# PKU-Alignment/Safe-Policy-Optimization

Hardware: NVIDIA H100
Metric: env-steps/sec PPO-Lag SafetyPointGoal1 @1024 envs/GPU (higher is better)
Workload: dtype f32

## Files before the change

### safe-policy-optimization_b200/csrc/spo_update_kernel.cuh

```cuda
#pragma once
#include <cooperative_groups.h>
#include <stdlib.h>
#include "spo_common.cuh"
#include "spo_mma.cuh"

namespace cg = cooperative_groups;

int spo_update_tile_pool(cudaMemPool_t* pool);

#ifdef SPO_PHASE_TIMERS
__device__ unsigned long long g_phase_cycles[16][24];
#define PHASE_MARK(idx)                                                   \
  do {                                                                    \
    if (tid == 0) {                                                       \
      const long long now__ = clock64();                                  \
      sm_phase__[idx] += static_cast<unsigned long long>(now__ - phase_t__); \
      phase_t__ = now__;                                                  \
    }                                                                     \
  } while (0)
#else
#define PHASE_MARK(idx) do { } while (0)
#endif

namespace {

constexpr int UT = 256;
constexpr int NQ = 4;
constexpr int SL = SPO_HID / NQ;
constexpr int NCTA = 3 * NQ;
constexpr int LDA = 72;
constexpr int LDS = 40;
constexpr float kLogSqrt2Pi = 0.91893853320467274178f;

template <int AC>
struct UpdShape {
  static_assert(AC == 8 || AC == 16, "action capacity 8 or 16");
  static constexpr int AUXW = 3 * AC + 4;
  static constexpr int AUX_LOGP = AC, AUX_ADV = AC + 1, AUX_TGT = AC + 2, AUX_OMEAN = AC + 4, AUX_OSTD = 2 * AC + 4;
  static constexpr int SP_B1 = 0, SP_B2 = SL, SP_W3 = 2 * SL, SP_B3 = 2 * SL + AC * SL, SP_LS = SP_B3 + AC;
  static constexpr int SPN = SP_LS + AC;
  static constexpr int SPT = (SPN + UT - 1) / UT;
  static constexpr int YQ = SPO_ROWS * AC;
  static constexpr int DH = AC / 4;
};
static_assert(UpdShape<8>::SPN == 176 && UpdShape<8>::SPT == 1 && UpdShape<16>::SPN == 320 && UpdShape<16>::SPT == 2, "layout");

__host__ __device__ constexpr int upd_ldx(int nt1) { return 64 * nt1 + 8; }
template <int NT1, int AC>
__host__ __device__ constexpr int upd_tile_floats() { return SPO_ROWS * (upd_ldx(NT1) + UpdShape<AC>::AUXW); }
static_assert(upd_tile_floats<1, 8>() * 4 == 25600 && upd_tile_floats<2, 8>() * 4 == 41984 && upd_tile_floats<2, 16>() * 4 % 16 == 0,
              "bulk copies move multiples of 16 bytes");
__host__ __device__ constexpr int dp_slot_words(int nt1) { return UT * 4 * (1 + nt1) + UT; }

template <int N> struct IC { static constexpr int value = N; };

struct UpdArgs {
  float *params, *adam_m, *adam_v;
  int* adam_t;
  float* tiles;
  spo_batch data;
  const int64_t* perm;
  int64_t perm_len;
  int batch, kind, D, A;
  int actor_only;
  spo_hparams hp;
  spo_update_ctrl* ctrl;
  spo_comm comm;
};

__device__ __forceinline__ uint32_t smem_u32(const void* p) { return static_cast<uint32_t>(__cvta_generic_to_shared(p)); }
__device__ __forceinline__ uint32_t mapa(uint32_t addr, uint32_t rank) {
  uint32_t r;
  asm volatile("mapa.shared::cluster.u32 %0, %1, %2;" : "=r"(r) : "r"(addr), "r"(rank));
  return r;
}
__device__ __forceinline__ void mbar_init(uint64_t* bar, uint32_t count) {
  asm volatile("mbarrier.init.shared::cta.b64 [%0], %1;" ::"r"(smem_u32(bar)), "r"(count) : "memory");
}
__device__ __forceinline__ void mbar_expect_tx(uint64_t* bar, uint32_t bytes) {
  asm volatile("mbarrier.arrive.expect_tx.shared::cta.b64 _, [%0], %1;" ::"r"(smem_u32(bar)), "r"(bytes) : "memory");
}
__device__ __forceinline__ void mbar_wait(uint64_t* bar, uint32_t parity) {
  const uint32_t a = smem_u32(bar);
  uint32_t ok = 0;
  while (!ok) {
    asm volatile("{ .reg .pred p; mbarrier.try_wait.parity.shared::cta.b64 p, [%1], %2; selp.u32 %0, 1, 0, p; }"
                 : "=r"(ok) : "r"(a), "r"(parity) : "memory");
  }
}
__device__ __forceinline__ void mbar_wait_cluster(uint64_t* bar, uint32_t parity) {
  const uint32_t a = smem_u32(bar);
  uint32_t ok = 0;
  while (!ok) {
    asm volatile("{ .reg .pred p; mbarrier.try_wait.parity.acquire.cluster.shared::cta.b64 p, [%1], %2; selp.u32 %0, 1, 0, p; }"
                 : "=r"(ok) : "r"(a), "r"(parity) : "memory");
  }
}
__device__ __forceinline__ void st_async16(uint32_t remote_dst, float4 v, uint32_t remote_bar) {
  asm volatile("st.async.shared::cluster.mbarrier::complete_tx::bytes.v4.b32 [%0], {%1, %2, %3, %4}, [%5];"
               ::"r"(remote_dst), "r"(__float_as_uint(v.x)), "r"(__float_as_uint(v.y)), "r"(__float_as_uint(v.z)),
               "r"(__float_as_uint(v.w)), "r"(remote_bar) : "memory");
}
__device__ __forceinline__ void bulk_push(uint32_t remote_dst, const void* local_src, uint32_t bytes, uint32_t remote_bar) {
  asm volatile("cp.async.bulk.shared::cluster.shared::cta.mbarrier::complete_tx::bytes [%0], [%1], %2, [%3];"
               ::"r"(remote_dst), "r"(smem_u32(local_src)), "r"(bytes), "r"(remote_bar) : "memory");
}
__device__ __forceinline__ void fence_proxy_async() { asm volatile("fence.proxy.async.shared::cta;" ::: "memory"); }
__device__ __forceinline__ void bulk_load(void* smem_dst, const void* gmem_src, uint32_t bytes, uint64_t* bar) {
  asm volatile("cp.async.bulk.shared::cluster.global.mbarrier::complete_tx::bytes [%0], [%1], %2, [%3];"
               ::"r"(smem_u32(smem_dst)), "l"(gmem_src), "r"(bytes), "r"(smem_u32(bar)) : "memory");
}
__device__ __forceinline__ void bulk_prefetch_l2(const void* gmem_src, uint32_t bytes) {
  asm volatile("cp.async.bulk.prefetch.L2.global [%0], %1;" ::"l"(gmem_src), "r"(bytes) : "memory");
}
__device__ __forceinline__ void st_ll(float2* p, float v, unsigned seq) {
  asm volatile("st.relaxed.sys.global.v2.b32 [%0], {%1, %2};" ::"l"(p), "r"(__float_as_uint(v)), "r"(seq) : "memory");
}

struct AdamK {
  float w1, b2, w2, ibc2s, eps, ss;
};
__device__ __forceinline__ float sqrt_approx(float x) {
  float r;
  asm("sqrt.approx.f32 %0, %1;" : "=f"(r) : "f"(x));
  return r;
}
__device__ __forceinline__ float adam_update(float p, float g, float& m, float& v, const AdamK& k) {
  m = fmaf(k.w1, __fsub_rn(g, m), m);
  v = __fadd_rn(__fmul_rn(v, k.b2), __fmul_rn(__fmul_rn(k.w2, g), g));
  const float denom = fmaf(sqrt_approx(v), k.ibc2s, k.eps);
  return __fadd_rn(p, __fdividef(__fmul_rn(k.ss, m), denom));
}

template <int NTL, int KSTEPS, bool ACCUM>
__device__ __forceinline__ void warp_gemm(float (&acc)[NTL][4], const float* __restrict__ A, int a_sm, int a_sk,
                                          const float* __restrict__ B, int b_sk, int b_sn, int m0, int n0) {
  const int lane = threadIdx.x & 31, g = lane >> 2, t = lane & 3;
  const float* a_ptr = A + (m0 + g) * a_sm + t * a_sk;
  const float* b_ptr = B + t * b_sk + (n0 + g) * b_sn;
  float c_lh[NTL][4], c_hl[NTL][4], c_hh[NTL][4];
#pragma unroll
  for (int nt = 0; nt < NTL; ++nt)
#pragma unroll
    for (int e = 0; e < 4; ++e) { c_lh[nt][e] = 0.f; c_hl[nt][e] = 0.f; c_hh[nt][e] = 0.f; }
  constexpr int CH = KSTEPS < 8 ? KSTEPS : 8;
#pragma unroll
  for (int kc = 0; kc < KSTEPS; kc += CH) {
    float af[CH][4], bf[CH][NTL][2];
#pragma unroll
    for (int ks = 0; ks < CH; ++ks) {
      const float* p = a_ptr + (kc + ks) * 8 * a_sk;
      af[ks][0] = p[0]; af[ks][1] = p[8 * a_sm]; af[ks][2] = p[4 * a_sk]; af[ks][3] = p[8 * a_sm + 4 * a_sk];
#pragma unroll
      for (int nt = 0; nt < NTL; ++nt) {
        const float* pb = b_ptr + nt * 8 * b_sn + (kc + ks) * 8 * b_sk;
        bf[ks][nt][0] = pb[0]; bf[ks][nt][1] = pb[4 * b_sk];
      }
    }
#pragma unroll
    for (int ks = 0; ks < CH; ++ks) {
      uint32_t ah[4], al[4];
#pragma unroll
      for (int i = 0; i < 4; ++i) spo_split_tf32(af[ks][i], ah[i], al[i]);
#pragma unroll
      for (int nt = 0; nt < NTL; ++nt) {
        uint32_t bh[2], bl[2];
        spo_split_tf32(bf[ks][nt][0], bh[0], bl[0]);
        spo_split_tf32(bf[ks][nt][1], bh[1], bl[1]);
        spo_mma_tf32(c_lh[nt], al, bh);
        spo_mma_tf32(c_hl[nt], ah, bl);
        spo_mma_tf32(c_hh[nt], ah, bh);
      }
    }
  }
#pragma unroll
  for (int nt = 0; nt < NTL; ++nt)
#pragma unroll
    for (int e = 0; e < 4; ++e) {
      const float s = (c_lh[nt][e] + c_hl[nt][e]) + c_hh[nt][e];
      acc[nt][e] = ACCUM ? acc[nt][e] + s : s;
    }
}

template <int KSTEPS>
__device__ __forceinline__ void warp_gemm_kk(float (&acc)[1][4], const float* __restrict__ A, int lda,
                                             const float* __restrict__ B, int ldb, int m0, int n0) {
  const int lane = threadIdx.x & 31, g = lane >> 2, t = lane & 3;
  const float* a_ptr = A + (m0 + g) * lda + 2 * t;
  const float* b_ptr = B + (n0 + g) * ldb + 2 * t;
  float c_lh[4] = {0.f, 0.f, 0.f, 0.f}, c_hl[4] = {0.f, 0.f, 0.f, 0.f}, c_hh[4] = {0.f, 0.f, 0.f, 0.f};
  constexpr int CH = KSTEPS < 8 ? KSTEPS : 8;
#pragma unroll
  for (int kc = 0; kc < KSTEPS; kc += CH) {
    float2 a0[CH], a1[CH], bb[CH];
#pragma unroll
    for (int ks = 0; ks < CH; ++ks) {
      a0[ks] = *reinterpret_cast<const float2*>(a_ptr + (kc + ks) * 8);
      a1[ks] = *reinterpret_cast<const float2*>(a_ptr + 8 * lda + (kc + ks) * 8);
      bb[ks] = *reinterpret_cast<const float2*>(b_ptr + (kc + ks) * 8);
    }
#pragma unroll
    for (int ks = 0; ks < CH; ++ks) {
      uint32_t ah[4], al[4], bh[2], bl[2];
      spo_split_tf32(a0[ks].x, ah[0], al[0]);
      spo_split_tf32(a1[ks].x, ah[1], al[1]);
      spo_split_tf32(a0[ks].y, ah[2], al[2]);
      spo_split_tf32(a1[ks].y, ah[3], al[3]);
      spo_split_tf32(bb[ks].x, bh[0], bl[0]);
      spo_split_tf32(bb[ks].y, bh[1], bl[1]);
      spo_mma_tf32(c_lh, al, bh);
      spo_mma_tf32(c_hl, ah, bl);
      spo_mma_tf32(c_hh, ah, bh);
    }
  }
#pragma unroll
  for (int e = 0; e < 4; ++e) acc[0][e] = (c_lh[e] + c_hl[e]) + c_hh[e];
}

constexpr int H1Q = SPO_ROWS * SL;

__device__ __forceinline__ void warp_gemm_l2(float (&acc)[1][4], const float* __restrict__ h1, const float* __restrict__ B, int ldb, int m0, int n0) {
  const int lane = threadIdx.x & 31, g = lane >> 2, t = lane & 3;
  const int r0 = m0 + g, sw = ((r0 >> 1) & 1) << 3;
  const float* b_ptr = B + (n0 + g) * ldb + 2 * t;
  float c_lh[4] = {0.f, 0.f, 0.f, 0.f}, c_hl[4] = {0.f, 0.f, 0.f, 0.f}, c_hh[4] = {0.f, 0.f, 0.f, 0.f};
  float2 a0[8], a1[8], bb[8];
#pragma unroll
  for (int ks = 0; ks < 8; ++ks) {
    const float* blk = h1 + (ks >> 1) * H1Q + ((((ks & 1) << 3) + 2 * t) ^ sw);
    a0[ks] = *reinterpret_cast<const float2*>(blk + r0 * SL);
    a1[ks] = *reinterpret_cast<const float2*>(blk + (r0 + 8) * SL);
    bb[ks] = *reinterpret_cast<const float2*>(b_ptr + ks * 8);
  }
#pragma unroll
  for (int ks = 0; ks < 8; ++ks) {
    uint32_t ah[4], al[4], bh[2], bl[2];
    spo_split_tf32(a0[ks].x, ah[0], al[0]);
    spo_split_tf32(a1[ks].x, ah[1], al[1]);
    spo_split_tf32(a0[ks].y, ah[2], al[2]);
    spo_split_tf32(a1[ks].y, ah[3], al[3]);
    spo_split_tf32(bb[ks].x, bh[0], bl[0]);
    spo_split_tf32(bb[ks].y, bh[1], bl[1]);
    spo_mma_tf32(c_lh, al, bh);
    spo_mma_tf32(c_hl, ah, bl);
    spo_mma_tf32(c_hh, ah, bh);
  }
#pragma unroll
  for (int e = 0; e < 4; ++e) acc[0][e] = (c_lh[e] + c_hl[e]) + c_hh[e];
}

__device__ __forceinline__ void warp_gemm_dw2(float (&acc)[1][4], const float* __restrict__ dz, int ldz, const float* __restrict__ h1, int n0) {
  const int lane = threadIdx.x & 31, g = lane >> 2, t = lane & 3;
  const float* a_ptr = dz + t * ldz + g;
  const int n = n0 + g, sw = ((t >> 1) & 1) << 3;
  const float* b_ptr = h1 + (n >> 4) * H1Q + t * SL + ((n & 15) ^ sw);
  float c_lh[4] = {0.f, 0.f, 0.f, 0.f}, c_hl[4] = {0.f, 0.f, 0.f, 0.f}, c_hh[4] = {0.f, 0.f, 0.f, 0.f};
  float af[8][4], bf[8][2];
#pragma unroll
  for (int ks = 0; ks < 8; ++ks) {
    const float* p = a_ptr + ks * 8 * ldz;
    af[ks][0] = p[0]; af[ks][1] = p[8]; af[ks][2] = p[4 * ldz]; af[ks][3] = p[4 * ldz + 8];
    const float* pb = b_ptr + ks * 8 * SL;
    bf[ks][0] = pb[0]; bf[ks][1] = pb[4 * SL];
  }
#pragma unroll
  for (int ks = 0; ks < 8; ++ks) {
    uint32_t ah[4], al[4], bh[2], bl[2];
#pragma unroll
    for (int i = 0; i < 4; ++i) spo_split_tf32(af[ks][i], ah[i], al[i]);
    spo_split_tf32(bf[ks][0], bh[0], bl[0]);
    spo_split_tf32(bf[ks][1], bh[1], bl[1]);
    spo_mma_tf32(c_lh, al, bh);
    spo_mma_tf32(c_hl, ah, bl);
    spo_mma_tf32(c_hh, ah, bh);
  }
#pragma unroll
  for (int e = 0; e < 4; ++e) acc[0][e] += (c_lh[e] + c_hl[e]) + c_hh[e];
}

template <int NT1, int AC>
__host__ __device__ constexpr size_t update_fixed_smem_bytes() {
  using S = UpdShape<AC>;
  return sizeof(float) * (4 * AC + 16 + SL * upd_ldx(NT1) + SL * LDA + 2 * S::SPN + NQ * SPO_ROWS * SL + 3 * SPO_ROWS * LDS +
                          (3 + NQ) * SPO_ROWS * AC + 2 * NQ * SPO_ROWS * SL + 64 + 128 + 3 * (4 * NT1 + 1) * UT);
}
template <int NT1, int AC>
__host__ __device__ constexpr int update_nslot() {
  return update_fixed_smem_bytes<NT1, AC>() + 2 * sizeof(float) * upd_tile_floats<NT1, AC>() <= 227 * 1024 ? 2 : 1;
}
template <int NT1, int AC>
__host__ __device__ constexpr size_t update_smem_bytes() {
  return update_fixed_smem_bytes<NT1, AC>() + update_nslot<NT1, AC>() * sizeof(float) * upd_tile_floats<NT1, AC>();
}
static_assert(update_smem_bytes<1, 8>() == 172352 && update_smem_bytes<2, 8>() == 221504 && update_smem_bytes<1, 16>() == 200256 &&
              update_smem_bytes<2, 16>() == 201280, "shared-memory figures in the comment above");

template <int NT1, int AC>
__global__ void __launch_bounds__(256) spo_pack_tiles(const UpdArgs a, int64_t n_tiles) {
  using S = UpdShape<AC>;
  if (*reinterpret_cast<volatile int*>(&a.ctrl->stop)) return;
  constexpr int ldx = upd_ldx(NT1), AUXW = S::AUXW, TILEF = upd_tile_floats<NT1, AC>();
  const int D = a.D, A = a.A, lane = threadIdx.x & 31;
  const int tps = (a.batch + SPO_ROWS - 1) / SPO_ROWS;
  const bool actor = a.kind != SPO_LOSS_CRITIC_ONLY, focops = a.kind == SPO_LOSS_FOCOPS;
  const int64_t n_rows = n_tiles * SPO_ROWS, wstride = (static_cast<int64_t>(gridDim.x) * blockDim.x) >> 5;
  for (int64_t w = (static_cast<int64_t>(blockIdx.x) * blockDim.x + threadIdx.x) >> 5; w < n_rows; w += wstride) {
    const int64_t t = w / SPO_ROWS, step = t / tps;
    const int r = static_cast<int>(w - t * SPO_ROWS), row = static_cast<int>(t - step * tps) * SPO_ROWS + r;
    int64_t rows_step = a.perm_len - step * a.batch;
    if (rows_step > a.batch) rows_step = a.batch;
    const bool valid = row < rows_step;
    const int64_t g = valid ? a.perm[step * a.batch + row] : 0;
    float* xo = a.tiles + t * TILEF + r * ldx;
    float* ao = a.tiles + t * TILEF + SPO_ROWS * ldx + r * AUXW;
    const float* xs = a.data.obs + g * D;
    for (int c = lane; c < ldx; c += 32) xo[c] = (valid && c < D) ? xs[c] : 0.f;
    for (int c = lane; c < AUXW; c += 32) {
      const float* src = nullptr;
      int64_t i = g;
      if (c < A) { if (actor) { src = a.data.act; i = g * A + c; } }
      else if (c == S::AUX_LOGP) { if (actor) src = a.data.logp; }
      else if (c == S::AUX_ADV) { if (actor) src = a.data.adv; }
      else if (c == S::AUX_TGT) src = a.data.target_r;
      else if (c == S::AUX_TGT + 1) src = a.data.target_c;
      else if (c >= S::AUX_OMEAN && c < S::AUX_OMEAN + A) { if (focops) { src = a.data.old_mean; i = g * A + c - S::AUX_OMEAN; } }
      else if (c >= S::AUX_OSTD && c < S::AUX_OSTD + A) { if (focops) { src = a.data.old_std; i = g * A + c - S::AUX_OSTD; } }
      ao[c] = (valid && src) ? src[i] : 0.f;
    }
  }
}

template <int NT1, int AC, bool DP>
__global__ void __launch_bounds__(UT, 1) spo_update_kernel(const UpdArgs a) {
  static_assert(!(DP && AC != 8), "the cross-GPU gradient slots hold one small parameter per thread");
  using S = UpdShape<AC>;
  constexpr int AUXW = S::AUXW, AUX_LOGP = S::AUX_LOGP, AUX_ADV = S::AUX_ADV, AUX_TGT = S::AUX_TGT, AUX_OMEAN = S::AUX_OMEAN,
                AUX_OSTD = S::AUX_OSTD;
  constexpr int SP_B1 = S::SP_B1, SP_B2 = S::SP_B2, SP_W3 = S::SP_W3, SP_B3 = S::SP_B3, SP_LS = S::SP_LS, SPN = S::SPN;
  constexpr int SPT = S::SPT, YQ = S::YQ, DH = S::DH;
  constexpr int NSLOT = update_nslot<NT1, AC>(), TILEF = upd_tile_floats<NT1, AC>();
  constexpr uint32_t TILEB = TILEF * sizeof(float);
  extern __shared__ __align__(16) float smem[];
  __shared__ __align__(8) uint64_t bar_h1, bar_dh, bar_y, bar_ss[2];
  __shared__ __align__(8) uint64_t bar_tile[NSLOT];
  __shared__ int comm_dead;
  cg::cluster_group cluster = cg::this_cluster();
  const unsigned rank = cluster.block_rank();
  const int tid = threadIdx.x, lane = tid & 31, wid = tid >> 5;
  spo_update_ctrl* ctrl = a.ctrl;
  if (*reinterpret_cast<volatile int*>(&ctrl->stop)) return;

  const int D = a.D, A = a.A;
  constexpr int ldx = upd_ldx(NT1);
  const bool idle = rank >= NCTA;
  const int net = idle ? 2 : static_cast<int>(rank) / NQ;
  const int q = static_cast<int>(rank) % NQ;
  const unsigned grp0 = static_cast<unsigned>(net * NQ);
  const bool is_actor = (net == 0);
  const bool active = !idle && !(is_actor && a.kind == SPO_LOSS_CRITIC_ONLY) && !(!is_actor && a.actor_only);
  const SpoNetOff off = spo_net_off(D, A, net);
  const int O = off.out;
  const int g8 = lane >> 2, t4 = lane & 3;

  float* p = smem;
  float* lsc = p; p += 4 * AC;
  float* adk = p; p += 16;
  float* w1s = p; p += SL * ldx;
  float* w2s = p; p += SL * LDA;
  float* sp = p;  p += SPN;
  float* gsmall = p; p += SPN;
  float* slots = p; p += NSLOT * TILEF;
  float* x = slots;
  float* aux = x + SPO_ROWS * ldx;
  float* h1 = p;  p += NQ * H1Q;
  float* h2s = p; p += SPO_ROWS * LDS;
  float* dz2s = p; p += SPO_ROWS * LDS;
  float* dz1s = p; p += SPO_ROWS * LDS;
  float* yblk = p; p += NQ * YQ;
  float* y = p;   p += SPO_ROWS * AC;
  float* dy = p;  p += SPO_ROWS * AC;
  float* dls = p; p += SPO_ROWS * AC;
  float* dh1b = p; p += NQ * H1Q;
  float* dh1in = p; p += NQ * H1Q;
  float* red = p; p += 64;
  float* bk = p;  p += 3 * (4 * NT1 + 1) * UT;
  float* xin = p; p += 2 * 16 * 4;
  float* b1s = sp + SP_B1; float* b2s = sp + SP_B2; float* w3s = sp + SP_W3; float* b3 = sp + SP_B3; float* log_std = sp + SP_LS;

  const int tps = (a.batch + SPO_ROWS - 1) / SPO_ROWS;
  const int64_t n_steps = (a.perm_len + a.batch - 1) / a.batch;
  const int64_t n_tiles = n_steps * tps;
  auto issue_tile = [&](int64_t t) {
    if (t >= n_tiles) return;
    const int s = static_cast<int>(t % NSLOT);
    mbar_expect_tx(&bar_tile[s], TILEB);
    bulk_load(slots + s * TILEF, a.tiles + t * TILEF, TILEB, &bar_tile[s]);
    if (NSLOT == 1 && t + 1 < n_tiles) bulk_prefetch_l2(a.tiles + (t + 1) * TILEF, TILEB);
  };

  if (tid == 0) {
    comm_dead = 0;
    mbar_init(&bar_h1, 1);
    mbar_init(&bar_dh, 1);
    mbar_init(&bar_y, 1);
    mbar_init(&bar_ss[0], 1);
    mbar_init(&bar_ss[1], 1);
#pragma unroll
    for (int s = 0; s < NSLOT; ++s) mbar_init(&bar_tile[s], 1);
    asm volatile("fence.mbarrier_init.release.cluster;" ::: "memory");
    if (!idle) { mbar_expect_tx(&bar_ss[0], (NCTA - 1) * 16); mbar_expect_tx(&bar_ss[1], (NCTA - 1) * 16); }
    for (int b = 0; b < 2; ++b) {
      adk[8 * b + 0] = static_cast<float>(1.0 - static_cast<double>(a.hp.beta1));
      adk[8 * b + 1] = a.hp.beta2;
      adk[8 * b + 2] = static_cast<float>(1.0 - static_cast<double>(a.hp.beta2));
      adk[8 * b + 4] = a.hp.adam_eps;
    }
    if (active) {
      mbar_expect_tx(&bar_h1, (NQ - 1) * H1Q * 4);
      mbar_expect_tx(&bar_dh, (NQ - 1) * H1Q * 4);
      mbar_expect_tx(&bar_y, (NQ - 1) * YQ * 4);
#pragma unroll
      for (int t = 0; t < NSLOT; ++t) issue_tile(t);
    }
  }

  bool sp_valid = false, sp_counted = false;
  int sp_goff = 0;
  if (tid < SPN && !idle) {
    const int i = tid;
    sp_counted = true;
    if (i < SP_B2) { sp_valid = true; sp_goff = off.b1 + SL * q + i; }
    else if (i < SP_W3) { sp_valid = true; sp_goff = off.b2 + SL * q + (i - SP_B2); }
    else if (i < SP_B3) { const int o = (i - SP_W3) / SL, kk = (i - SP_W3) % SL; sp_valid = o < O; sp_goff = off.w3 + o * SPO_HID + SL * q + kk; }
    else if (i < SP_LS) { const int o = i - SP_B3; sp_valid = o < O; sp_goff = off.b3 + o; sp_counted = (q == 0); }
    else { const int j = i - SP_LS; sp_valid = is_actor && j < A; sp_goff = off.log_std + j; sp_counted = (q == 0); }
  }
  float sp_m = 0.f, sp_v = 0.f;
  bool sp_valid1 = false, sp_counted1 = false;
  int sp_goff1 = 0;
  float sp_m1 = 0.f, sp_v1 = 0.f;
  if constexpr (SPT > 1) {
    static_assert(UT > SP_W3, "entry 1 lies past b1 / b2");
    const int i = tid + UT;
    if (i < SPN && !idle) {
      sp_counted1 = true;
      if (i < SP_B3) { const int o = (i - SP_W3) / SL, kk = (i - SP_W3) % SL; sp_valid1 = o < O; sp_goff1 = off.w3 + o * SPO_HID + SL * q + kk; }
      else if (i < SP_LS) { const int o = i - SP_B3; sp_valid1 = o < O; sp_goff1 = off.b3 + o; sp_counted1 = (q == 0); }
      else { const int j = i - SP_LS; sp_valid1 = is_actor && j < A; sp_goff1 = off.log_std + j; sp_counted1 = (q == 0); }
    }
  }

  if (!idle) {
    for (int i = tid; i < SL * ldx; i += UT) {
      const int j = i / ldx, k = i - j * ldx;
      w1s[i] = (k < D) ? __ldg(a.params + off.w1 + (SL * q + j) * D + k) : 0.f;
    }
    for (int i = tid; i < SL * LDA; i += UT) {
      const int j = i / LDA, k = i - j * LDA;
      w2s[i] = (k < SPO_HID) ? __ldg(a.params + off.w2 + (SL * q + j) * SPO_HID + k) : 0.f;
    }
    if (tid < SPN) {
      sp[tid] = sp_valid ? a.params[sp_goff] : 0.f;
      gsmall[tid] = 0.f;
      if (sp_valid) { sp_m = a.adam_m[sp_goff]; sp_v = a.adam_v[sp_goff]; }
    }
    if constexpr (SPT > 1) {
      if (tid + UT < SPN) {
        sp[tid + UT] = sp_valid1 ? a.params[sp_goff1] : 0.f;
        gsmall[tid + UT] = 0.f;
        if (sp_valid1) { sp_m1 = a.adam_m[sp_goff1]; sp_v1 = a.adam_v[sp_goff1]; }
      }
    }
  }
  float mW2[4], vW2[4], mW1[NT1][4], vW1[NT1][4];
  auto frag_jk = [&](int e, int ntile, int& j, int& k) { j = g8 + ((e >> 1) << 3); k = 8 * ntile + 2 * t4 + (e & 1); };
#pragma unroll
  for (int e = 0; e < 4; ++e) {
    int j, k;
    frag_jk(e, wid, j, k);
    mW2[e] = active ? a.adam_m[off.w2 + (SL * q + j) * SPO_HID + k] : 0.f;
    vW2[e] = active ? a.adam_v[off.w2 + (SL * q + j) * SPO_HID + k] : 0.f;
#pragma unroll
    for (int i = 0; i < NT1; ++i) {
      frag_jk(e, wid + 8 * i, j, k);
// ... 177 lines not shown
        vW1[i][e] = bk[(2 * NWB + 4 * i + e) * UT + tid];
      }
    }
    if (tid < SP_B2) {
      sp[tid] = bk[(0 * NWB + NWB - 1) * UT + tid];
      sp_m = bk[(1 * NWB + NWB - 1) * UT + tid];
      sp_v = bk[(2 * NWB + NWB - 1) * UT + tid];
    }
  };
  auto clear_l1_grads = [&]() {
#pragma unroll
    for (int e = 0; e < 4; ++e)
#pragma unroll
      for (int i = 0; i < NT1; ++i) gW1[i][e] = 0.f;
    if (tid < SP_B2) gsmall[tid] = 0.f;
  };
  auto set_lsc = [&](int j, float ls) {
    const float sd = expf(ls);
    lsc[4 * j + 0] = sd;
    lsc[4 * j + 1] = __fdiv_rn(1.f, __fmul_rn(sd, sd));
    lsc[4 * j + 2] = logf(sd);
  };
  auto adam_rest = [&](float clip, const AdamK& k) {
    float2 w2v[2];
    float spv = 0.f, spg = 0.f, spv1 = 0.f, spg1 = 0.f;
    const bool own0 = tid >= SP_B2 && tid < SPN;
#pragma unroll
    for (int e = 0; e < 4; e += 2) {
      int j, kc;
      frag_jk(e, wid, j, kc);
      w2v[e >> 1] = *reinterpret_cast<const float2*>(w2s + j * LDA + kc);
    }
    if (own0) { spv = sp[tid]; spg = gsmall[tid]; }
    if constexpr (SPT > 1) {
      if (tid + UT < SPN) { spv1 = sp[tid + UT]; spg1 = gsmall[tid + UT]; }
    }
#pragma unroll
    for (int e = 0; e < 4; e += 2) {
      w2v[e >> 1].x = adam_update(w2v[e >> 1].x, __fmul_rn(gW2[0][e], clip), mW2[e], vW2[e], k);
      w2v[e >> 1].y = adam_update(w2v[e >> 1].y, __fmul_rn(gW2[0][e + 1], clip), mW2[e + 1], vW2[e + 1], k);
    }
    if (own0 && sp_valid) {
      spv = adam_update(spv, __fmul_rn(spg, clip), sp_m, sp_v, k);
      if (tid >= SP_LS) set_lsc(tid - SP_LS, spv);
    }
    if constexpr (SPT > 1) {
      if (tid + UT < SPN && sp_valid1) {
        spv1 = adam_update(spv1, __fmul_rn(spg1, clip), sp_m1, sp_v1, k);
        if (tid + UT >= SP_LS) set_lsc(tid + UT - SP_LS, spv1);
      }
    }
#pragma unroll
    for (int e = 0; e < 4; e += 2) {
      int j, kc;
      frag_jk(e, wid, j, kc);
      *reinterpret_cast<float2*>(w2s + j * LDA + kc) = w2v[e >> 1];
    }
    if (own0) { sp[tid] = spv; gsmall[tid] = 0.f; }
    if constexpr (SPT > 1) {
      if (tid + UT < SPN) { sp[tid + UT] = spv1; gsmall[tid + UT] = 0.f; }
    }
#pragma unroll
    for (int e = 0; e < 4; ++e) gW2[0][e] = 0.f;
  };

  int64_t step = 0;
  int sub = 0;
  auto next_tile = [&]() { if (++sub == tps) { sub = 0; ++step; } };
  for (int64_t qt = 0; qt < n_tiles; ++qt, next_tile()) {
    x = slots + (qt % NSLOT) * TILEF;
    aux = x + SPO_ROWS * ldx;
    int64_t rs64 = a.perm_len - step * a.batch;
    if (rs64 > a.batch) rs64 = a.batch;
    const int rows_step = static_cast<int>(rs64);
    int rows = rows_step - sub * SPO_ROWS;
    rows = rows < 0 ? 0 : (rows > SPO_ROWS ? SPO_ROWS : rows);
    const bool last_tile = (sub == tps - 1);
    const float inv_b = __fdiv_rn(1.f, static_cast<float>(rows_step));
    const unsigned seq = static_cast<unsigned>(a.comm.seq_base + static_cast<unsigned long long>(step_idx) + 1ull);
    const int par = static_cast<int>(step_idx & 1);
    auto dp_push = [&](const float* vals, auto n_c, int w0) {
      constexpr int n = decltype(n_c)::value;
      const size_t base = ((static_cast<size_t>(seq & 1u) * world + me) * NCTA + rank) * DPW;
      for (int r = 0; r < world; ++r) {
        if (r == me) continue;
        float2* dst = reinterpret_cast<float2*>(a.comm.grad_bufs[r]) + base;
#pragma unroll
        for (int i = 0; i < n; ++i) st_ll(dst + (w0 + i) * UT + tid, vals[i], seq);
      }
    };
    auto dp_sum_wide = [&](float (&g2)[4], float (&g1)[NT1][4], float& gs) {
      constexpr int NW = 4 * (1 + NT1) + 1, G = 3;
      const unsigned limit = a.comm.spin_limit ? a.comm.spin_limit : 400000000u;
      const float inv_w = __fdiv_rn(1.f, static_cast<float>(world));
      float val[NW];
#pragma unroll
      for (int e = 0; e < 4; ++e) {
        val[e] = g2[e];
#pragma unroll
        for (int i = 0; i < NT1; ++i) val[4 * (1 + i) + e] = g1[i][e];
      }
      val[NW - 1] = gs;
      const float2* slot0 = reinterpret_cast<const float2*>(a.comm.grad_bufs[me]) + (static_cast<size_t>(seq & 1u) * world * NCTA + rank) * DPW + tid;
      const size_t rstride = static_cast<size_t>(NCTA) * DPW;
#pragma unroll
      for (int i0 = 0; i0 < NW; i0 += G) {
        unsigned need = 0;
#pragma unroll
        for (int j = 0; j < G; ++j)
          if (i0 + j < NW && ((i0 + j < NW - 1) || tid < SPN))
#pragma unroll
            for (int r = 0; r < 8; ++r)
              if (r < world && r != me) need |= 1u << (r * G + j);
        unsigned got = 0, polls = 0;
        float v[8][G];
        while (got != need) {
          unsigned wa[8][G], wb[8][G];
#pragma unroll
          for (int r = 0; r < 8; ++r)
#pragma unroll
            for (int j = 0; j < G; ++j)
              if (((need & ~got) >> (r * G + j)) & 1u)
                asm volatile("ld.relaxed.sys.global.v2.b32 {%0, %1}, [%2];" : "=r"(wa[r][j]), "=r"(wb[r][j]) : "l"(slot0 + r * rstride + (i0 + j) * UT) : "memory");
#pragma unroll
          for (int r = 0; r < 8; ++r)
#pragma unroll
            for (int j = 0; j < G; ++j)
              if ((((need & ~got) >> (r * G + j)) & 1u) && wb[r][j] == seq) { v[r][j] = __uint_as_float(wa[r][j]); got |= 1u << (r * G + j); }
          if (got != need) {
            if (*reinterpret_cast<volatile int*>(&comm_dead)) break;
            if (++polls > limit) { comm_dead = 1; atomicExch(&ctrl->stop, 2); break; }
          }
        }
#pragma unroll
        for (int j = 0; j < G; ++j)
          if (i0 + j < NW) {
            float acc = 0.f;
#pragma unroll
            for (int r = 0; r < 8; ++r)
              if (r < world) acc += (r == me) ? val[i0 + j] : (((got >> (r * G + j)) & 1u) ? v[r][j] : 0.f);
            val[i0 + j] = __fmul_rn(acc, inv_w);
          }
      }
#pragma unroll
      for (int e = 0; e < 4; ++e) {
        g2[e] = val[e];
#pragma unroll
        for (int i = 0; i < NT1; ++i) g1[i][e] = val[4 * (1 + i) + e];
      }
      gs = val[NW - 1];
    };
    auto dp_sum_all = [&](float (&g2)[4], float (&g1)[NT1][4], float& gs) {
      constexpr int NW = 4 * (1 + NT1) + 1;
      const unsigned limit = a.comm.spin_limit ? a.comm.spin_limit : 400000000u;
      const unsigned need = (tid < SPN) ? ((1u << NW) - 1u) : ((1u << (NW - 1)) - 1u);
      float acc[NW];
#pragma unroll
      for (int i = 0; i < NW; ++i) acc[i] = 0.f;
      for (int r = 0; r < world; ++r) {
        if (r == me) {
#pragma unroll
          for (int e = 0; e < 4; ++e) {
            acc[e] += g2[e];
#pragma unroll
            for (int i = 0; i < NT1; ++i) acc[4 * (1 + i) + e] += g1[i][e];
          }
          acc[NW - 1] += gs;
          continue;
        }
        const float2* src = reinterpret_cast<const float2*>(a.comm.grad_bufs[me]) + ((static_cast<size_t>(seq & 1u) * world + r) * NCTA + rank) * DPW + tid;
        unsigned got = 0, polls = 0;
        float v[NW];
#pragma unroll
        for (int i = 0; i < NW; ++i) v[i] = 0.f;
        while (got != need) {
          unsigned wa[NW], wb[NW];
#pragma unroll
          for (int i = 0; i < NW; ++i)
            if (!((got >> i) & 1u) && ((need >> i) & 1u))
              asm volatile("ld.relaxed.sys.global.v2.b32 {%0, %1}, [%2];" : "=r"(wa[i]), "=r"(wb[i]) : "l"(src + i * UT) : "memory");
#pragma unroll
          for (int i = 0; i < NW; ++i)
            if (!((got >> i) & 1u) && ((need >> i) & 1u) && wb[i] == seq) { v[i] = __uint_as_float(wa[i]); got |= 1u << i; }
          if (got != need) {
            if (*reinterpret_cast<volatile int*>(&comm_dead)) break;
            if (++polls > limit) { comm_dead = 1; atomicExch(&ctrl->stop, 2); break; }
          }
        }
#pragma unroll
        for (int i = 0; i < NW; ++i) acc[i] += v[i];
      }
      const float inv_w = __fdiv_rn(1.f, static_cast<float>(world));
#pragma unroll
      for (int e = 0; e < 4; ++e) {
        g2[e] = __fmul_rn(acc[e], inv_w);
#pragma unroll
        for (int i = 0; i < NT1; ++i) g1[i][e] = __fmul_rn(acc[4 * (1 + i) + e], inv_w);
      }
      gs = __fmul_rn(acc[NW - 1], inv_w);
    };

    if (active) mbar_wait(&bar_tile[qt % NSLOT], static_cast<uint32_t>(qt / NSLOT) & 1u);
    __syncthreads();
    PHASE_MARK(0);

    if (active) layer1();
    PHASE_MARK(2);
    const bool defer = pending;
    float clip = 1.f;
    if (pending) {
      pending = false;
      step_barrier_wait();
      PHASE_MARK(9);
      clip = resolve_clip(pend_par);
      if (active) {
        if (clip < 1.f) {
          __syncthreads();
          adam_l1_restore();
          adam_l1(clip, false, adam_k(pend_par));
          __syncthreads();
          layer1();
        }
        clear_l1_grads();
      }
    }
    PHASE_MARK(1);
    float yv[AC];
    if (active) {
      __syncthreads();
      if (lane == 0 && wid < NQ && wid != q)
        bulk_push(mapa(smem_u32(h1 + q * H1Q), grp0 + wid), h1 + q * H1Q, H1Q * 4, mapa(smem_u32(&bar_h1), grp0 + wid));
      if (defer) {
        adam_rest(clip, adam_k(pend_par));
        __syncthreads();
      } else if (qt == 0 && is_actor && tid >= UT - 32 && tid - (UT - 32) < A) {
        set_lsc(tid - (UT - 32), log_std[tid - (UT - 32)]);
      }
      PHASE_MARK(19);
      mbar_wait(&bar_h1, ph_x);
      if (tid == 0) mbar_expect_tx(&bar_h1, (NQ - 1) * H1Q * 4);
      PHASE_MARK(3);
      {
        float acc[1][4];
        warp_gemm_l2(acc, h1, w2s, LDA, mt * 16, ntl * 8);
        const float2 bb = *reinterpret_cast<const float2*>(b2s + cA);
        *reinterpret_cast<float2*>(h2s + rA * LDS + cA) = make_float2(spo_tanh_fast(acc[0][0] + bb.x), spo_tanh_fast(acc[0][1] + bb.y));
        *reinterpret_cast<float2*>(h2s + (rA + 8) * LDS + cA) = make_float2(spo_tanh_fast(acc[0][2] + bb.x), spo_tanh_fast(acc[0][3] + bb.y));
      }
      __syncthreads();
      {
        const float4 hv = *reinterpret_cast<const float4*>(h2s + r4 * LDS + 4 * k4);
        for (int o = 0; o < O; o += 2) {
          const float4 wa = *reinterpret_cast<const float4*>(w3s + o * SL + 4 * k4);
          const float4 wb = *reinterpret_cast<const float4*>(w3s + (o + 1) * SL + 4 * k4);
          float sa = fmaf(hv.x, wa.x, hv.y * wa.y) + fmaf(hv.z, wa.z, hv.w * wa.w);
          float sb = fmaf(hv.x, wb.x, hv.y * wb.y) + fmaf(hv.z, wb.z, hv.w * wb.w);
          sa += __shfl_xor_sync(0xffffffffu, sa, 1);
          sb += __shfl_xor_sync(0xffffffffu, sb, 1);
          sa += __shfl_xor_sync(0xffffffffu, sa, 2);
          sb += __shfl_xor_sync(0xffffffffu, sb, 2);
          if (k4 == (o & 3)) yblk[q * YQ + r4 * AC + o] = sa;
          if (k4 == ((o + 1) & 3) && o + 1 < O) yblk[q * YQ + r4 * AC + o + 1] = sb;
        }
        fence_proxy_async();
      }
      __syncthreads();
      if (lane == 0 && wid < NQ && wid != q)
        bulk_push(mapa(smem_u32(yblk + q * YQ), grp0 + wid), yblk + q * YQ, YQ * 4, mapa(smem_u32(&bar_y), grp0 + wid));
      PHASE_MARK(4);
      float pa[DH], psd[DH], piv[DH], pls[DH], plogp = 0.f, padv = 0.f, ptgt = 0.f;
#pragma unroll
      for (int h = 0; h < DH; ++h) pa[h] = 0.f;
#pragma unroll
      for (int h = 0; h < DH; ++h) psd[h] = 1.f;
#pragma unroll
      for (int h = 0; h < DH; ++h) piv[h] = 1.f;
#pragma unroll
      for (int h = 0; h < DH; ++h) pls[h] = 0.f;
      {
        const float* axp = aux + r4 * AUXW;
        if (is_actor) {
#pragma unroll
          for (int h = 0; h < DH; ++h) {
            const int j = k4 + 4 * h;
            if (j < A) { pa[h] = axp[j]; psd[h] = lsc[4 * j]; piv[h] = lsc[4 * j + 1]; pls[h] = lsc[4 * j + 2]; }
          }
          plogp = axp[AUX_LOGP];
          padv = axp[AUX_ADV];
        } else if (k4 == 0) {
          ptgt = axp[AUX_TGT + (net == 2 ? 1 : 0)];
        }
      }
      if (defer) log_loss(pend_par, pend_inv_b);
      if (last_tile) {
        float* kp = adk + 8 * par;
        if (tid == UT - 32) {
          b1pow *= static_cast<double>(a.hp.beta1);
          kp[5] = -__fdiv_rn(lr, static_cast<float>(1.0 - b1pow));
        } else if (tid == UT - 64) {
          b2pow *= static_cast<double>(a.hp.beta2);
          kp[3] = __fdiv_rn(1.f, sqrtf(static_cast<float>(1.0 - b2pow)));
        }
      }
      mbar_wait(&bar_y, ph_x);
      if (tid == 0) mbar_expect_tx(&bar_y, (NQ - 1) * YQ * 4);
      PHASE_MARK(5);
      {
        const float4* yp = reinterpret_cast<const float4*>(yblk + k4 * YQ + r4 * AC);
#pragma unroll
        for (int c = 0; c < AC / 4; ++c) {
          float4 v = make_float4(0.f, 0.f, 0.f, 0.f);
          if (c == 0 || O > 4 * c) v = yp[c];
          yv[4 * c] = v.x; yv[4 * c + 1] = v.y; yv[4 * c + 2] = v.z; yv[4 * c + 3] = v.w;
        }
#pragma unroll
        for (int o = 0; o < AC; ++o) {
          if (o < O) {
            yv[o] += __shfl_xor_sync(0xffffffffu, yv[o], 1);
            yv[o] += __shfl_xor_sync(0xffffffffu, yv[o], 2);
            yv[o] = __fadd_rn(yv[o], b3[o]);
          }
        }
      }
      float part0 = 0.f, part1 = 0.f, part2 = 0.f;
      {
        const int r = r4;
        const bool valid = r < rows;
        float* ax = aux + r * AUXW;
        if (!is_actor) {
          if (k4 == 0) {
            const float dv = __fsub_rn(yv[0], ptgt);
            part0 = valid ? __fmul_rn(dv, dv) : 0.f;
            dy[r * AC] = valid ? __fmul_rn(__fmul_rn(__fmul_rn(2.f, dv), inv_b), vcoef) : 0.f;
          }
        } else {
          float term[DH], klj[DH], dmu_lp[DH], dls_lp[DH], dmu_kl[DH], dls_kl[DH];
#pragma unroll
          for (int h = 0; h < DH; ++h) term[h] = 0.f;
#pragma unroll
          for (int h = 0; h < DH; ++h) klj[h] = 0.f;
#pragma unroll
          for (int h = 0; h < DH; ++h) dmu_kl[h] = 0.f;
#pragma unroll
          for (int h = 0; h < DH; ++h) dls_kl[h] = 0.f;
#pragma unroll
          for (int h = 0; h < DH; ++h) {
            const int j = k4 + 4 * h;
            dmu_lp[h] = 0.f; dls_lp[h] = 0.f;
            if (j < A) {
              float mean;
              if constexpr (DH == 2) {
                const float m_lo = (k4 == 0) ? yv[0] : (k4 == 1) ? yv[1] : (k4 == 2) ? yv[2] : yv[3];
                const float m_hi = (k4 == 0) ? yv[4] : (k4 == 1) ? yv[5] : (k4 == 2) ? yv[6] : yv[7];
                mean = h ? m_hi : m_lo;
              } else {
                mean = (k4 == 0) ? yv[4 * h] : (k4 == 1) ? yv[4 * h + 1] : (k4 == 2) ? yv[4 * h + 2] : yv[4 * h + 3];
              }
              const float std = psd[h], inv_var = piv[h];
              const float diff = __fsub_rn(pa[h], mean);
              const float d2 = __fmul_rn(diff, diff);
              const float q2 = __fmul_rn(d2, inv_var);
              term[h] = __fsub_rn(__fsub_rn(__fmul_rn(-0.5f, q2), pls[h]), kLogSqrt2Pi);
              dmu_lp[h] = __fmul_rn(diff, inv_var);
              dls_lp[h] = __fsub_rn(q2, 1.f);
              if (a.kind == SPO_LOSS_FOCOPS) {
                const float os = valid ? ax[AUX_OSTD + j] : 1.f, om = ax[AUX_OMEAN + j];
                const float ios = __fdiv_rn(1.f, os);
                const float sr = __fmul_rn(std, ios);
                const float vr = __fmul_rn(sr, sr);
                const float dm = __fmul_rn(__fsub_rn(mean, om), ios);
                const float t1 = __fmul_rn(dm, dm);
                klj[h] = __fmul_rn(0.5f, __fsub_rn(__fsub_rn(__fadd_rn(vr, t1), 1.f), logf(vr)));
                dmu_kl[h] = __fmul_rn(dm, ios);
                dls_kl[h] = __fsub_rn(vr, 1.f);
              }
            }
          }
          float lp = term[0], kl = klj[0];
#pragma unroll
          for (int h = 1; h < DH; ++h) { lp += term[h]; kl += klj[h]; }
          lp += __shfl_xor_sync(0xffffffffu, lp, 1);
          lp += __shfl_xor_sync(0xffffffffu, lp, 2);
          if (a.kind == SPO_LOSS_FOCOPS) {
            kl += __shfl_xor_sync(0xffffffffu, kl, 1);
            kl += __shfl_xor_sync(0xffffffffu, kl, 2);
          }
          const float ratio = expf(__fsub_rn(lp, plogp));
          const float adv = padv;
          if (a.kind == SPO_LOSS_PPO_CLIP) {
            const float s1 = __fmul_rn(ratio, adv);
            const float s2 = __fmul_rn(fminf(fmaxf(ratio, a.hp.clip_lo), a.hp.clip_hi), adv);
            if (k4 == 0) part0 = valid ? -fminf(s1, s2) : 0.f;
            const float gl = (valid && s1 <= s2) ? -__fmul_rn(__fmul_rn(adv, ratio), inv_b) : 0.f;
#pragma unroll
            for (int h = 0; h < DH; ++h) {
              const int j = k4 + 4 * h;
              if (j < A) {
                dy[r * AC + j] = __fmul_rn(gl, dmu_lp[h]);
                dls[r * AC + j] = __fmul_rn(gl, dls_lp[h]);
              }
            }
          } else {
            const float mask = (valid && kl <= a.hp.focops_kl) ? 1.f : 0.f;
            if (k4 == 0) {
              part0 = valid ? __fmul_rn(kl, mask) : 0.f;
              part1 = valid ? __fmul_rn(ratio, adv) : 0.f;
              part2 = mask;
            }
            const float gl = valid ? __fmul_rn(__fmul_rn(adv, ratio), inv_b) : 0.f;
#pragma unroll
            for (int h = 0; h < DH; ++h) {
              const int j = k4 + 4 * h;
              if (j < A) {
                dy[r * AC + j] = __fmul_rn(__fmul_rn(mask, inv_b), dmu_kl[h]);
                dls[r * AC + j] = __fmul_rn(__fmul_rn(mask, inv_b), dls_kl[h]);
                y[r * AC + j] = __fmul_rn(gl, dmu_lp[h]);
                ax[AUX_OMEAN + j] = __fmul_rn(gl, dls_lp[h]);
              }
            }
          }
        }
        part0 = spo_warp_sum(part0);
        if (is_actor && a.kind == SPO_LOSS_FOCOPS) { part1 = spo_warp_sum(part1); part2 = spo_warp_sum(part2); }
        if (lane == 0) { red[wid * 4 + 0] = part0; red[wid * 4 + 1] = part1; red[wid * 4 + 2] = part2; }
      }
      __syncthreads();
      if (is_actor && a.kind == SPO_LOSS_FOCOPS) {
        float msum = 0.f;
#pragma unroll
        for (int w = 0; w < UT / 32; ++w) msum += red[w * 4 + 2];
        const float mbar = __fmul_rn(msum, inv_b);
        const float c2 = -__fmul_rn(__fdiv_rn(1.f, a.hp.focops_lam), mbar);
        const float* ax = aux + r4 * AUXW;
#pragma unroll
        for (int h = 0; h < DH; ++h) {
          const int j = k4 + 4 * h;
          if (j < A) {
            dy[r4 * AC + j] = __fadd_rn(dy[r4 * AC + j], __fmul_rn(c2, y[r4 * AC + j]));
            dls[r4 * AC + j] = __fadd_rn(dls[r4 * AC + j], __fmul_rn(c2, ax[AUX_OMEAN + j]));
          }
        }
        __syncthreads();
      }
      PHASE_MARK(6);

      {
        float4 s4 = make_float4(0.f, 0.f, 0.f, 0.f);
        for (int o = 0; o < O; ++o) {
          const float d = dy[r4 * AC + o];
          const float4 wv = *reinterpret_cast<const float4*>(w3s + o * SL + 4 * k4);
          s4.x = fmaf(d, wv.x, s4.x); s4.y = fmaf(d, wv.y, s4.y); s4.z = fmaf(d, wv.z, s4.z); s4.w = fmaf(d, wv.w, s4.w);
        }
        const float4 h = *reinterpret_cast<const float4*>(h2s + r4 * LDS + 4 * k4);
        s4.x *= (1.f - h.x * h.x); s4.y *= (1.f - h.y * h.y); s4.z *= (1.f - h.z * h.z); s4.w *= (1.f - h.w * h.w);
        *reinterpret_cast<float4*>(dz2s + r4 * LDS + 4 * k4) = s4;
      }
      __syncthreads();
      PHASE_MARK(7);
      {
        float acc[4][4];
        warp_gemm<4, 2, false>(acc, dz2s, LDS, 1, w2s, LDA, 1, mt * 16, (wid >> 2) * 32);
#pragma unroll
        for (int nt = 0; nt < 4; ++nt) {
          const int c = (wid >> 2) * 32 + nt * 8 + 2 * t4;
          float* blk = dh1b + (c >> 4) * H1Q + (c & 15);
          *reinterpret_cast<float2*>(blk + rA * SL) = make_float2(acc[nt][0], acc[nt][1]);
          *reinterpret_cast<float2*>(blk + (rA + 8) * SL) = make_float2(acc[nt][2], acc[nt][3]);
        }
        fence_proxy_async();
      }
      __syncthreads();
      if (lane == 0 && wid < NQ && wid != q)
        bulk_push(mapa(smem_u32(dh1in + q * H1Q), grp0 + wid), dh1b + wid * H1Q, H1Q * 4, mapa(smem_u32(&bar_dh), grp0 + wid));
      PHASE_MARK(8);
      if (tid == 0) {
        float l0 = 0.f, l1 = 0.f, l2 = 0.f;
#pragma unroll
        for (int w = 0; w < UT / 32; ++w) { l0 += red[w * 4]; l1 += red[w * 4 + 1]; l2 += red[w * 4 + 2]; }
        step_loss += l0;
        step_aux0 += l1;
        step_aux1 += l2;
      }
      warp_gemm_dw2(gW2, dz2s, LDS, h1, wid * 8);
      colsum_into(dz2s, gsmall + SP_B2);
      PHASE_MARK(10);
      {
        const int kk = tid >> 4, rg = tid & 15;
        float hv[4];
#pragma unroll
        for (int i = 0; i < 4; ++i) hv[i] = h2s[(rg + 16 * i) * LDS + kk];
        if constexpr (AC == 8) {
          const int col = kk & 7;
          const bool need = (kk < 8) ? (col < O) : (is_actor && col < A);
          const float* src = (kk < 8) ? dy : dls;
          float sc = 0.f;
          if (need) {
#pragma unroll
            for (int i = 0; i < 4; ++i) sc += src[(rg + 16 * i) * AC + col];
          }
          for (int o = 0; o < O; o += 2) {
            float sa = 0.f, sb = 0.f;
#pragma unroll
            for (int i = 0; i < 4; ++i) {
              const float2 d = *reinterpret_cast<const float2*>(dy + (rg + 16 * i) * AC + o);
              sa = fmaf(d.x, hv[i], sa);
              sb = fmaf(d.y, hv[i], sb);
            }
#pragma unroll
            for (int m = 1; m < 16; m <<= 1) {
              sa += __shfl_xor_sync(0xffffffffu, sa, m);
              sb += __shfl_xor_sync(0xffffffffu, sb, m);
              if (o == 0) sc += __shfl_xor_sync(0xffffffffu, sc, m);
            }
            if (rg == 0) {
              gsmall[SP_W3 + o * SL + kk] += sa;
              if (o + 1 < O) gsmall[SP_W3 + (o + 1) * SL + kk] += sb;
            }
          }
          if (need && rg == 0) gsmall[(kk < 8 ? SP_B3 : SP_LS) + col] += sc;
        } else {
          const bool need_b3 = kk < O, need_ls = is_actor && kk < A;
          float sc = 0.f, sl = 0.f;
#pragma unroll
          for (int i = 0; i < 4; ++i) {
            if (need_b3) sc += dy[(rg + 16 * i) * AC + kk];
            if (need_ls) sl += dls[(rg + 16 * i) * AC + kk];
          }
          for (int o = 0; o < O; o += 2) {
            float sa = 0.f, sb = 0.f;
#pragma unroll
            for (int i = 0; i < 4; ++i) {
              const float2 d = *reinterpret_cast<const float2*>(dy + (rg + 16 * i) * AC + o);
              sa = fmaf(d.x, hv[i], sa);
              sb = fmaf(d.y, hv[i], sb);
            }
#pragma unroll
            for (int m = 1; m < 16; m <<= 1) {
              sa += __shfl_xor_sync(0xffffffffu, sa, m);
              sb += __shfl_xor_sync(0xffffffffu, sb, m);
              if (o == 0) { sc += __shfl_xor_sync(0xffffffffu, sc, m); sl += __shfl_xor_sync(0xffffffffu, sl, m); }
            }
            if (rg == 0) {
              gsmall[SP_W3 + o * SL + kk] += sa;
              if (o + 1 < O) gsmall[SP_W3 + (o + 1) * SL + kk] += sb;
            }
          }
          if (rg == 0) {
            if (need_b3) gsmall[SP_B3 + kk] += sc;
            if (need_ls) gsmall[SP_LS + kk] += sl;
          }
        }
      }
      PHASE_MARK(20);
      if (DP && world > 1 && last_tile) {
        __syncthreads();
        float sv = (tid >= SP_B2 && tid < SPN) ? gsmall[tid] : 0.f;
        dp_push(gW2[0], IC<4>{}, 0);
        if (tid >= SP_B2 && tid < SPN) dp_push(&sv, IC<1>{}, 4 * (1 + NT1));
      }
      mbar_wait(&bar_dh, ph_x);
      if (tid == 0) mbar_expect_tx(&bar_dh, (NQ - 1) * H1Q * 4);
      {
        float4 v[NQ];
#pragma unroll
        for (int d = 0; d < NQ; ++d) {
          const float* src = (d == q) ? dh1b + q * H1Q : dh1in + d * H1Q;
          v[d] = *reinterpret_cast<const float4*>(src + r4 * SL + 4 * k4);
        }
        float4 s4 = v[0];
#pragma unroll
        for (int d = 1; d < NQ; ++d) { s4.x += v[d].x; s4.y += v[d].y; s4.z += v[d].z; s4.w += v[d].w; }
        const float4 h = *reinterpret_cast<const float4*>(h1 + q * H1Q + r4 * SL + ((4 * k4) ^ (((r4 >> 1) & 1) << 3)));
        s4.x *= (1.f - h.x * h.x); s4.y *= (1.f - h.y * h.y); s4.z *= (1.f - h.z * h.z); s4.w *= (1.f - h.w * h.w);
        *reinterpret_cast<float4*>(dz1s + r4 * LDS + 4 * k4) = s4;
      }
      __syncthreads();
      PHASE_MARK(11);
#pragma unroll
      for (int i = 0; i < NT1; ++i)
        warp_gemm<1, 8, true>(reinterpret_cast<float (&)[1][4]>(gW1[i]), dz1s, 1, LDS, x, ldx, 1, 0, (wid + 8 * i) * 8);
      colsum_into(dz1s, gsmall + SP_B1);
      fence_proxy_async();
      PHASE_MARK(12);
    }

    __syncthreads();
    if (active && tid == UT - 32) issue_tile(qt + NSLOT);
    ph_x ^= active ? 1u : 0u;
    if (!last_tile) {
      step_barrier_push(par, 0.f, 0.f);
      step_barrier_wait();
      continue;
    }

    if (DP && world > 1 && active) {
      float sv = 0.f;
      if (tid < SP_B2) { sv = gsmall[tid]; dp_push(&sv, IC<1>{}, 4 * (1 + NT1)); }
#pragma unroll
      for (int i = 0; i < NT1; ++i) dp_push(gW1[i], IC<4>{}, 4 * (1 + i));
      sv = (tid < SPN) ? gsmall[tid] : 0.f;
      if (world >= 4 && world <= 8) dp_sum_wide(gW2[0], gW1, sv);
      else dp_sum_all(gW2[0], gW1, sv);
      if (tid < SPN) gsmall[tid] = sv;
    }
    PHASE_MARK(13);

    if (active) {
      float ss = 0.f, th2 = 0.f;
#pragma unroll
      for (int e = 0; e < 4; ++e) {
        int j, k;
        frag_jk(e, wid, j, k);
        if (!is_actor) {
          const float th = w2s[j * LDA + k];
          gW2[0][e] = fmaf(reg, th, gW2[0][e]);
          th2 = fmaf(th, th, th2);
        }
        ss = fmaf(gW2[0][e], gW2[0][e], ss);
#pragma unroll
        for (int i = 0; i < NT1; ++i) {
          frag_jk(e, wid + 8 * i, j, k);
          if (k < D) {
            if (!is_actor) {
              const float t1 = w1s[j * ldx + k];
              gW1[i][e] = fmaf(reg, t1, gW1[i][e]);
              th2 = fmaf(t1, t1, th2);
            }
            ss = fmaf(gW1[i][e], gW1[i][e], ss);
          } else {
            gW1[i][e] = 0.f;
          }
        }
      }
      if (tid < SPN && sp_valid) {
        const float th = sp[tid];
        const float g = fmaf(reg, th, gsmall[tid]);
        gsmall[tid] = g;
        if (sp_counted) { ss = fmaf(g, g, ss); th2 = fmaf(th, th, th2); }
      }
      if constexpr (SPT > 1) {
        if (tid + UT < SPN && sp_valid1) {
          const float th = sp[tid + UT];
          const float g = fmaf(reg, th, gsmall[tid + UT]);
          gsmall[tid + UT] = g;
          if (sp_counted1) { ss = fmaf(g, g, ss); th2 = fmaf(th, th, th2); }
        }
      }
      ss = spo_warp_sum(ss);
      if (!is_actor) th2 = spo_warp_sum(th2);
      if (lane == 0) *reinterpret_cast<float2*>(red + 16 + 2 * wid) = make_float2(ss, th2);
      __syncthreads();
    }
    {
      float s = 0.f, t2 = 0.f;
      if (tid < NCTA && active) {
#pragma unroll
        for (int w = 0; w < UT / 32; w += 2) {
          const float4 v = *reinterpret_cast<const float4*>(red + 16 + 2 * w);
          s += v.x + v.z; t2 += v.y + v.w;
        }
      }
      PHASE_MARK(14);
      step_barrier_push(par, s + extra_sumsq, t2);
      PHASE_MARK(17);
    }
    if (active) adam_l1(1.f, true, adam_k(par));
    pending = true;
    pend_par = par;
    pend_inv_b = inv_b;
    PHASE_MARK(16);
    ++step_idx;
  }
  if (pending) {
    __syncthreads();
    step_barrier_wait();
    const float clip = resolve_clip(pend_par);
    if (active) {
      if (clip < 1.f) {
        __syncthreads();
        adam_l1_restore();
        adam_l1(clip, false, adam_k(pend_par));
      }
      log_loss(pend_par, pend_inv_b);
      adam_rest(clip, adam_k(pend_par));
    }
  }
  __syncthreads();

  if (active) {
    for (int i = tid; i < SL * D; i += UT) {
      const int j = i / D, kx = i - j * D;
      a.params[off.w1 + (SL * q + j) * D + kx] = w1s[j * ldx + kx];
    }
    for (int i = tid; i < SL * SPO_HID; i += UT)
      a.params[off.w2 + (SL * q + (i >> 6)) * SPO_HID + (i & 63)] = w2s[(i >> 6) * LDA + (i & 63)];
    if (tid < SPN && sp_valid && (sp_counted || tid < SP_B3)) {
      a.params[sp_goff] = sp[tid];
      a.adam_m[sp_goff] = sp_m;
      a.adam_v[sp_goff] = sp_v;
    }
    if constexpr (SPT > 1) {
      if (tid + UT < SPN && sp_valid1 && (sp_counted1 || tid + UT < SP_B3)) {
        a.params[sp_goff1] = sp[tid + UT];
        a.adam_m[sp_goff1] = sp_m1;
        a.adam_v[sp_goff1] = sp_v1;
      }
    }
#pragma unroll
    for (int e = 0; e < 4; ++e) {
      int j, kc;
      frag_jk(e, wid, j, kc);
      a.adam_m[off.w2 + (SL * q + j) * SPO_HID + kc] = mW2[e];
      a.adam_v[off.w2 + (SL * q + j) * SPO_HID + kc] = vW2[e];
#pragma unroll
      for (int i = 0; i < NT1; ++i) {
        frag_jk(e, wid + 8 * i, j, kc);
        if (kc < D) {
          a.adam_m[off.w1 + (SL * q + j) * D + kc] = mW1[i][e];
          a.adam_v[off.w1 + (SL * q + j) * D + kc] = vW1[i][e];
        }
      }
    }
    if (tid == 0 && q == 0) {
      a.adam_t[net] = t0 + static_cast<int>(n_steps);
      const int slot = (net == 0) ? 2 : (net == 1 ? 0 : 1);
      atomicAdd(&ctrl->loss_sum[slot], acc_loss);
    }
  }
#ifdef SPO_PHASE_TIMERS
  if (tid < 24) atomicAdd(&g_phase_cycles[rank & 15][tid], sm_phase__[tid]);
#endif
  if (rank == NQ && tid == 0) atomicAdd(reinterpret_cast<unsigned long long*>(&ctrl->steps), static_cast<unsigned long long>(n_steps));
  cluster.sync();
}

inline int64_t upd_n_tiles(const UpdArgs& a) {
  return (a.perm_len + a.batch - 1) / a.batch * ((a.batch + SPO_ROWS - 1) / SPO_ROWS);
}

template <int NT1, int AC>
int launch_pack(const UpdArgs& a, cudaStream_t stream) {
  const int64_t n_tiles = upd_n_tiles(a);
  const int64_t blocks = (n_tiles * SPO_ROWS + 7) / 8;
  spo_pack_tiles<NT1, AC><<<static_cast<unsigned>(blocks < 65536 ? blocks : 65536), 256, 0, stream>>>(a, n_tiles);
  SPO_CUDA_TRY(cudaGetLastError());
  return SPO_OK;
}

template <int NT1, int AC, bool DP>
int launch_update_kernel(const UpdArgs& a, cudaStream_t stream) {
  constexpr size_t smem = update_smem_bytes<NT1, AC>();
  static_assert(smem <= 227 * 1024, "shared memory of the update kernel");
  static int cluster_size = 0;
  SPO_CUDA_TRY(cudaFuncSetAttribute(spo_update_kernel<NT1, AC, DP>, cudaFuncAttributeMaxDynamicSharedMemorySize, static_cast<int>(smem)));
  SPO_CUDA_TRY(cudaFuncSetAttribute(spo_update_kernel<NT1, AC, DP>, cudaFuncAttributeNonPortableClusterSizeAllowed, 1));
  if (!cluster_size) {
    const char* env = getenv("SPO_CLUSTER");
    if (env && atoi(env) >= NCTA && atoi(env) <= 16) cluster_size = atoi(env);
  }
  for (int attempt = 0; attempt < 2; ++attempt) {
    const int cs = cluster_size ? cluster_size : (attempt == 0 ? NCTA : 16);
    cudaLaunchConfig_t cfg{};
    cfg.gridDim = dim3(cs);
    cfg.blockDim = dim3(UT);
    cfg.dynamicSmemBytes = smem;
    cfg.stream = stream;
    cudaLaunchAttribute attr[1];
// ... 38 lines not shown
```

Baseline: 230,800.

## Compute dz2 in registers and feed MMA fragments directly, dropping barrier

Each warp now computes the dz2 backprop values it needs, laid out in the MMA A-fragment layout, directly in registers. The values go straight into a new specialized GEMM, so the shared-memory round-trip and the __syncthreads before the dh1 GEMM are gone. The tanh-derivative factor is also precomputed earlier, before the y barrier wait, to overlap with latency. The cost is redundant dz computation across warps that share rows, plus only a conditional store of dz2s for later use.

```diff
diff --git a/safe-policy-optimization_b200/csrc/spo_update_kernel.cuh b/safe-policy-optimization_b200/csrc/spo_update_kernel.cuh
--- a/safe-policy-optimization_b200/csrc/spo_update_kernel.cuh
+++ b/safe-policy-optimization_b200/csrc/spo_update_kernel.cuh
@@ -180,6 +180,43 @@
       const float s = (c_lh[nt][e] + c_hl[nt][e]) + c_hh[nt][e];
       acc[nt][e] = ACCUM ? acc[nt][e] + s : s;
     }
+}
+
+__device__ __forceinline__ void warp_gemm_dh1(float (&acc)[4][4], const float (&af)[2][4], const float* __restrict__ B, int ldb, int n0) {
+  const int lane = threadIdx.x & 31, g = lane >> 2, t = lane & 3;
+  const float* b_ptr = B + t * ldb + n0 + g;
+  float bf[2][4][2];
+#pragma unroll
+  for (int ks = 0; ks < 2; ++ks)
+#pragma unroll
+    for (int nt = 0; nt < 4; ++nt) {
+      const float* pb = b_ptr + nt * 8 + ks * 8 * ldb;
+      bf[ks][nt][0] = pb[0]; bf[ks][nt][1] = pb[4 * ldb];
+    }
+  float c_lh[4][4], c_hl[4][4], c_hh[4][4];
+#pragma unroll
+  for (int nt = 0; nt < 4; ++nt)
+#pragma unroll
+    for (int e = 0; e < 4; ++e) { c_lh[nt][e] = 0.f; c_hl[nt][e] = 0.f; c_hh[nt][e] = 0.f; }
+#pragma unroll
+  for (int ks = 0; ks < 2; ++ks) {
+    uint32_t ah[4], al[4];
+#pragma unroll
+    for (int i = 0; i < 4; ++i) spo_split_tf32(af[ks][i], ah[i], al[i]);
+#pragma unroll
+    for (int nt = 0; nt < 4; ++nt) {
+      uint32_t bh[2], bl[2];
+      spo_split_tf32(bf[ks][nt][0], bh[0], bl[0]);
+      spo_split_tf32(bf[ks][nt][1], bh[1], bl[1]);
+      spo_mma_tf32(c_lh[nt], al, bh);
+      spo_mma_tf32(c_hl[nt], ah, bl);
+      spo_mma_tf32(c_hh[nt], ah, bh);
+    }
+  }
+#pragma unroll
+  for (int nt = 0; nt < 4; ++nt)
+#pragma unroll
+    for (int e = 0; e < 4; ++e) acc[nt][e] = (c_lh[nt][e] + c_hl[nt][e]) + c_hh[nt][e];
 }
 
 template <int KSTEPS>
@@ -963,6 +1000,14 @@
           kp[3] = __fdiv_rn(1.f, sqrtf(static_cast<float>(1.0 - b2pow)));
         }
       }
+      float dh2[2][4];
+#pragma unroll
+      for (int r = 0; r < 2; ++r)
+#pragma unroll
+        for (int i = 0; i < 4; ++i) {
+          const float h = h2s[(rA + 8 * r) * LDS + t4 + 4 * i];
+          dh2[r][i] = 1.f - h * h;
+        }
       mbar_wait(&bar_y, ph_x);
       if (tid == 0) mbar_expect_tx(&bar_y, (NQ - 1) * YQ * 4);
       PHASE_MARK(5);
@@ -1105,25 +1150,38 @@
       }
       PHASE_MARK(6);
 
+      float dz[2][4];
       {
-        float4 s4 = make_float4(0.f, 0.f, 0.f, 0.f);
-        for (int o = 0; o < O; ++o) {
-          const float d = dy[r4 * AC + o];
-          const float4 wv = *reinterpret_cast<const float4*>(w3s + o * SL + 4 * k4);
-          s4.x = fmaf(d, wv.x, s4.x); s4.y = fmaf(d, wv.y, s4.y); s4.z = fmaf(d, wv.z, s4.z); s4.w = fmaf(d, wv.w, s4.w);
-        }
-        const float4 h = *reinterpret_cast<const float4*>(h2s + r4 * LDS + 4 * k4);
-        s4.x *= (1.f - h.x * h.x); s4.y *= (1.f - h.y * h.y); s4.z *= (1.f - h.z * h.z); s4.w *= (1.f - h.w * h.w);
-        *reinterpret_cast<float4*>(dz2s + r4 * LDS + 4 * k4) = s4;
-      }
-      __syncthreads();
+#pragma unroll
+        for (int i = 0; i < 4; ++i) { dz[0][i] = 0.f; dz[1][i] = 0.f; }
+#pragma unroll
+        for (int o = 0; o < AC; ++o) {
+          if (o < O) {
+            const float d0 = dy[rA * AC + o], d8 = dy[(rA + 8) * AC + o];
+#pragma unroll
+            for (int i = 0; i < 4; ++i) {
+              const float w = w3s[o * SL + t4 + 4 * i];
+              dz[0][i] = fmaf(d0, w, dz[0][i]);
+              dz[1][i] = fmaf(d8, w, dz[1][i]);
+            }
+          }
+        }
+#pragma unroll
+        for (int r = 0; r < 2; ++r)
+#pragma unroll
+          for (int i = 0; i < 4; ++i) {
+            dz[r][i] *= dh2[r][i];
+            if (ntl == 0) dz2s[(rA + 8 * r) * LDS + t4 + 4 * i] = dz[r][i];
+          }
+      }
       PHASE_MARK(7);
       {
+        const float af[2][4] = {{dz[0][0], dz[1][0], dz[0][1], dz[1][1]}, {dz[0][2], dz[1][2], dz[0][3], dz[1][3]}};
         float acc[4][4];
-        warp_gemm<4, 2, false>(acc, dz2s, LDS, 1, w2s, LDA, 1, mt * 16, (wid >> 2) * 32);
+        warp_gemm_dh1(acc, af, w2s, LDA, ntl * 32);
 #pragma unroll
         for (int nt = 0; nt < 4; ++nt) {
-          const int c = (wid >> 2) * 32 + nt * 8 + 2 * t4;
+          const int c = ntl * 32 + nt * 8 + 2 * t4;
           float* blk = dh1b + (c >> 4) * H1Q + (c & 15);
           *reinterpret_cast<float2*>(blk + rA * SL) = make_float2(acc[nt][0], acc[nt][1]);
           *reinterpret_cast<float2*>(blk + (rA + 8) * SL) = make_float2(acc[nt][2], acc[nt][3]);
```

After: 233,900 (median of 6 runs). 1.01x the previous value.
